# danini/progressive-x

Measured on AMD Instinct MI355X. Metric: residual_evals_per_sec, higher is better.
Workload: dtype f64; 1 GPU; C4 multi-6D-pose points (1e6 2D-3D correspondences, 16 objects, 20% outliers) x metric batch of 2048 pose hypotheses (16 GT + perturbed; weak mode: per GPU), PnP reprojection residual, MSAC + compound-model score, compound instance = 1 model; points=1000000, points_per_gpu=1000000, hypotheses_per_gpu=2048, hypotheses_total=2048, parallelism=1 GPU, exchange=none, device=AMD GPU, 256 CUs (gfx950:sramecc+:xnack-), cu_count=256

## Files before the change

### progressive-x_amd/csrc/capi.hip

```cpp
#include <cmath>
#include <cstdarg>
#include <cstdlib>
#include <cstring>
#include <algorithm>
#include <vector>
#include <cmath>

#include "pgx_internal.h"

namespace pgx {

static thread_local std::string g_err;

int fail(pgx_ctx* ctx, int code, const char* fmt, ...)
{
    char buf[1024];
    va_list ap;
    va_start(ap, fmt);
    vsnprintf(buf, sizeof(buf), fmt, ap);
    va_end(ap);
    if (ctx) ctx->err = buf;
    g_err = buf;
    return code;
}
// ... 130 lines not shown
    if (e != hipSuccess || count <= 0)
        return fail(nullptr, PGX_ERR_HIP, "pgx_create: no HIP device available (%s)",
                    e != hipSuccess ? hipGetErrorString(e) : "device count is 0");
    if (device_id < 0 || device_id >= count)
        return fail(nullptr, PGX_ERR_INVALID, "pgx_create: device %d out of range [0,%d)", device_id, count);
    pgx_ctx* ctx = new pgx_ctx();
    ctx->device = device_id;
    if ((e = hipSetDevice(device_id)) != hipSuccess || (e = hipStreamCreate(&ctx->stream)) != hipSuccess ||
        (e = hipEventCreate(&ctx->ev0)) != hipSuccess || (e = hipEventCreate(&ctx->ev1)) != hipSuccess) {
        int r = fail(nullptr, PGX_ERR_HIP, "pgx_create: HIP init failed: %s", hipGetErrorString(e));
        delete ctx;
        return r;
    }
    hipDeviceProp_t prop;
    if (hipGetDeviceProperties(&prop, device_id) == hipSuccess) ctx->cu_count = prop.multiProcessorCount;
    const char* nf = std::getenv("PGX_NO_FILTER");
    ctx->score_sw.filter_enabled = (nf && nf[0] == '1') ? 0 : ((nf && nf[0] == '2') ? 2 : 1);
    if (const char* ns = std::getenv("PGX_NO_SORT")) ctx->score_sort = (ns[0] == '1') ? 0 : 1;
    if (const char* b = std::getenv("PGX_SP_KD")) { const int v = std::atoi(b); ctx->sp_kd = v < 0 ? 0 : (v > 2 ? 2 : v); }
    if (const char* b = std::getenv("PGX_SETPOINTS_HOST")) ctx->setpoints_host = std::atoi(b) ? 1 : 0;
    if (const char* b = std::getenv("PGX_GC_FLIP")) ctx->route.gc_flip = std::atoi(b) ? 1 : 0;
    if (const char* b = std::getenv("PGX_SCORE_MIRROR")) ctx->score_sw.mirror = std::atoi(b) != 0;
    if (const char* b = std::getenv("PGX_SCORE_NO_CULL")) ctx->score_sw.cull = std::atoi(b) ? 0 : 1;
    if (const char* b = std::getenv("PGX_NO_GROUP")) ctx->group_filter = std::atoi(b) ? 0 : 1;
    if (const char* b = std::getenv("PGX_VERIFY")) ctx->score_sw.verify = std::atoi(b) ? 1 : 0;
    if (const char* b = std::getenv("PGX_MF_TILE")) ctx->route.mf_tile = std::atoi(b) ? 1 : 0;
    if (const char* b = std::getenv("PGX_MF_TILE_BATCH")) ctx->route.mf_tile_batch = std::atoi(b) ? 1 : 0;
    if (const char* b = std::getenv("PGX_MF_REGION")) ctx->route.mf_region = std::atoi(b) ? 1 : 0;
    if (const char* b = std::getenv("PGX_MF_MEMO")) ctx->expansion.mf_memo = std::atoi(b) ? 1 : 0;
    if (const char* b = std::getenv("PGX_MF_DONE_VERIFY")) ctx->expansion.mf_done_verify = std::atoi(b) ? 1 : 0;
    if (const char* b = std::getenv("PGX_MF_XCD")) ctx->mf_xcd = std::atoi(b) ? 1 : 0;
    if (const char* b = std::getenv("PGX_MF_XCD_SEARCH")) ctx->mf_xcd_search = std::atoi(b) ? 1 : 0;
    if (const char* b = std::getenv("PGX_MF_XCD_MIN_DEPTH")) ctx->mf_xcd_min_depth = std::atoi(b);
    if (const char* b = std::getenv("PGX_MF_XCD_MAXN")) ctx->mf_xcd_max_n = std::atoll(b);
    if (const char* b = std::getenv("PGX_MF_SWEEPS")) ctx->mf_sweeps = std::atoi(b);
    if (const char* b = std::getenv("PGX_TILE_MINI")) ctx->tile_mini = std::atoi(b) ? 1 : 0;
    if (const char* b = std::getenv("PGX_TILE_EXPANSION_MAX")) { const int v = std::atoi(b); ctx->route.tile_expansion_max = v < 0 ? 0 : v; }
    if (const char* b = std::getenv("PGX_TILE_MINI_SWEEPS")) { const int v = std::atoi(b); ctx->tile_mini_sweeps = v < 1 ? 1 : v; }
    if (const char* b = std::getenv("PGX_MF_DEBUG")) ctx->tile_debug = std::atoi(b);
    *out = ctx;
    return PGX_OK;
}

void pgx_destroy(pgx_ctx* ctx)
{
    if (!ctx) return;
    (void)hipSetDevice(ctx->device);
    if (ctx->stream) (void)hipStreamSynchronize(ctx->stream);
    comm_free(ctx);
    maxflow_free(ctx);
    tile_free(ctx);
    release(ctx->gorder);
    DevBuf* bufs[] = {&ctx->pts, &ctx->comp, &ctx->pmax, &ctx->pts32, &ctx->perm, &ctx->models, &ctx->pcnt, &ctx->pval, &ctx->psh, &ctx->counts,
                      &ctx->masks, &ctx->g_counts, &ctx->g_values, &ctx->g_shared,
                      &ctx->red_partials, &ctx->red_out, &ctx->dq, &ctx->kmodels, &ctx->labels, &ctx->goff,
                      &ctx->gidx, &ctx->gmult, &ctx->grev, &ctx->scratch, &ctx->fit_scratch, &ctx->pts_s, &ctx->pts32_s,
                      &ctx->pmax_s, &ctx->comp_s, &ctx->pperm, &ctx->gbounds, &ctx->masks_s, &ctx->cull_lists, &ctx->cull_counts, &ctx->gc, &ctx->gc_sel,
                      &ctx->weights, &ctx->stats_buf, &ctx->pts_g, &ctx->p32_g, &ctx->weights_scratch, &ctx->memo_snaps.buf, &ctx->prosac_tops};
    for (DevBuf* b : bufs) release(*b);
    for (DevBuf& b : ctx->slots) release(b);
    release(ctx->h_res);
    release(ctx->h_mirror);
    ctx->h_samples.free();
    ctx->h_models.free();
    if (ctx->h_rb) (void)hipHostFree(ctx->h_rb);
    for (int k = 0; k < 5; ++k) if (ctx->kev[k]) (void)hipEventDestroy(ctx->kev[k]);
    if (ctx->ev0) (void)hipEventDestroy(ctx->ev0);
    if (ctx->ev1) (void)hipEventDestroy(ctx->ev1);
    if (ctx->stream) (void)hipStreamDestroy(ctx->stream);
    delete ctx;
}

const char* pgx_last_error(const pgx_ctx* ctx) { return ctx ? ctx->err.c_str() : g_err.c_str(); }

#define CTX_GUARD(ctx)                                                            \
    do {                                                                          \
        if (!(ctx)) return fail(nullptr, PGX_ERR_INVALID, "ctx is NULL");        \
        hipError_t e_ = hipSetDevice((ctx)->device);                              \
        if (e_ != hipSuccess) return fail(ctx, PGX_ERR_HIP, "hipSetDevice: %s", hipGetErrorString(e_)); \
        (ctx)->rb.clear();                                                        \
// ... 326 lines not shown
}

int pgx_score_algorithmic_bytes(pgx_ctx* ctx, int want_masks, int64_t* bytes, int64_t* pairs)
{
    if (!ctx || ctx->n <= 0 || ctx->batch.resident.M <= 0) return fail(ctx, PGX_ERR_INVALID, "pgx_score_algorithmic_bytes: nothing to score");
    const int64_t M = ctx->batch.resident.M;
    int64_t b = ctx->n * ctx->D * 8 + M * ctx->P * 8 + M * 16;
    if (ctx->batch.last.has_compound) b += ctx->n * 8;
    if (want_masks) b += M * ((ctx->n + 63) / 64) * 8;
    if (bytes) *bytes = b;
    if (pairs) *pairs = ctx->n * M;
    return PGX_OK;
}

int pgx_score_debug_geometry(pgx_ctx* ctx, int what, int value)
{
    CTX_GUARD(ctx);
    switch (what) {
    case 0: if (value < 0 || value > 1024) break; ctx->score_sw.split = value; return PGX_OK;
    case 1: if (value < -1 || value > 1) break; ctx->score_sw.group_xcd = value; return PGX_OK;
    case 2: if (value < 0 || value > 1024 || value % 8) break; ctx->score_sw.nrep = value; return PGX_OK;
    case 3: if (value < 1 || value > 65) break; ctx->score_sw.dense_min = value; return PGX_OK;
    case 4: if (value < 1 || value > 65535) break; ctx->score_sw.cull_segs = value; return PGX_OK;
    }
    return fail(ctx, PGX_ERR_INVALID, "pgx_score_debug_geometry: what = %d, value = %d out of range", what, value);
}

int pgx_score_debug_fetch(pgx_ctx* ctx, int what, void* out, int64_t bytes)
{
    CTX_GUARD(ctx);
    if (!out || bytes <= 0) return fail(ctx, PGX_ERR_INVALID, "pgx_score_debug_fetch: empty destination");
    if (!ctx->point_sort) return fail(ctx, PGX_ERR_INVALID, "pgx_score_debug_fetch: no sorted copies for the resident points");
    const int64_t groups = (ctx->n + 63) / 64, supers = (groups + kSuper - 1) / kSuper;
    if (what == 5) {
        const int64_t want = (int64_t)3 * ctx->batch.resident.Mpad * 8;
        if (bytes != want) return fail(ctx, PGX_ERR_INVALID, "pgx_score_debug_fetch: buffer 5 holds %lld bytes, asked for %lld", (long long)want, (long long)bytes);
        PGX_TRY(ensure(ctx, ctx->g_counts, (size_t)want));
        PGX_TRY(score_acc_export(ctx, (unsigned long long*)ctx->g_counts.p, ctx->stream));
        PGX_TRY(d2h(ctx, out, ctx->g_counts.p, (size_t)bytes));
        PGX_TRY(sync_deliver(ctx));
        return PGX_OK;
    }
    const DevBuf* b = nullptr;
    int64_t have = 0;
    switch (what) {
    case 0: b = &ctx->pperm; have = ctx->n * 4; break;
    case 1: b = &ctx->gbounds; have = (groups + supers) * kGroupRow * 4; break;
    case 2: b = &ctx->pts_g; have = groups * 64 * ctx->D * 8; break;
    case 3: b = &ctx->p32_g; have = groups * 64 * 8 * 4; break;
    case 4: b = &ctx->pts32_s; have = ctx->n * 8 * 4; break;
    default: return fail(ctx, PGX_ERR_INVALID, "pgx_score_debug_fetch: unknown buffer %d", what);
    }
    if (bytes != have) return fail(ctx, PGX_ERR_INVALID, "pgx_score_debug_fetch: buffer %d holds %lld bytes, asked for %lld", what, (long long)have, (long long)bytes);
    PGX_TRY(d2h(ctx, out, b->p, (size_t)bytes));
    PGX_TRY(sync_deliver(ctx));
    return PGX_OK;
}

int pgx_score_profile(pgx_ctx* ctx, int on)
{
    CTX_GUARD(ctx);
    if (on && !ctx->kev[0])
        for (int k = 0; k < 5; ++k) PGX_HIP(ctx, hipEventCreate(&ctx->kev[k]));
    ctx->score_profile = on < 0 ? 0 : (on > 2 ? 2 : on);
    return PGX_OK;
}

int pgx_score_kernel_times(pgx_ctx* ctx, float ms[4])
// ... 443 lines not shown
```

### progressive-x_amd/csrc/pgx_internal.h

```cpp
#pragma once
#include <hip/hip_runtime.h>

#include <cstdint>
#include <cstdio>
#include <string>
#include <vector>

#include "../../include/pgx.h"
#include "expansion_cycle.h"
#include "move_route.h"
#include "residuals.hip.h"
#include "score_plan.h"

namespace pgx {

struct StagedCopy { void* dst; size_t off, bytes; };
struct DevBuf {
    void* p = nullptr;
    size_t cap = 0;
    template <class T> T* as() const { return reinterpret_cast<T*>(p); }
};

struct PinnedBuf { void* p = nullptr; size_t cap = 0; };
struct PinnedStage {
// ... 20 lines not shown
    std::string err;
    int cu_count = 0;

    int model_type = -1, D = 0, P = 0;
    int64_t n = 0;
    pgx::DevBuf pts, comp;
    pgx::DevBuf pmax;
    pgx::DevBuf pts32;
    double umax = 0.0;
    double fscale = 0.0;
    double rmin = 0.0, rmax = __builtin_inf();
    pgx::ScoreSwitches score_sw;
    pgx::DevBuf stats_buf;
    int point_sort = 0;
    int group_filter = 1;
    int comp_dirty = 0;
    pgx::DevBuf pts_s, pts32_s, pmax_s, comp_s, pperm, gbounds, masks_s;
    pgx::DevBuf pts_g, p32_g;
    int setpoints_host = 0;
    double sp_kd_weight = 0.25;
    int sp_kd = 1;
    pgx::DevBuf weights_scratch;
    pgx::DevBuf cull_lists, cull_counts;
    pgx::DevBuf gc;
    pgx::DevBuf gc_sel;

    pgx::ScoreBatch batch;
    int64_t score_global_n = 0;
    pgx::DevBuf models, pcnt, pval, psh, counts, values, shared, masks;
    pgx::DevBuf perm;
    int score_sort = 1;
    pgx::DevBuf g_counts, g_values, g_shared;

    std::vector<pgx::DevBuf> slots;
    pgx::DevBuf red_partials, red_out;

    int L = 0;
    int64_t dq_n = 0;
    pgx::DevBuf dq;
    int64_t dq_max = 0;
    pgx::DevBuf kmodels;
    pgx::DevBuf labels;
    int64_t labels_n = 0;
    pgx::ExpansionState expansion;
    struct MemoSnapshots {
        pgx::DevBuf buf;
// ... 142 lines not shown
```

### progressive-x_amd/csrc/score.hip

```cpp
#include <cmath>
#include <cstdlib>

#include "pgx_internal.h"
#include "score_filters.hip.h"
#include "score_runs.h"

namespace pgx {


template <int MT, bool MASK, int FILT>
__global__ __launch_bounds__(kScoreBlock) void score_kernel(
    const double* __restrict__ pts, int64_t n, const double* __restrict__ models, int M, int Mpad,
    double T2, const double* __restrict__ comp, int has_comp, int64_t chunk,
    const double* __restrict__ pmax, double guard, const float* __restrict__ pts32, double guard32,
    unsigned* __restrict__ pcnt, double* __restrict__ pval, double* __restrict__ psh,
    unsigned long long* __restrict__ masks, int64_t words, const int* __restrict__ perm, int chunks, int xcd_map,
    const float* __restrict__ gbounds)
{
    using R = Residual<MT>;
    int gx = (int)blockIdx.x, gy = (int)blockIdx.y;
    if (xcd_map) {
        const int groups = Mpad / kScoreBlock;
        const int slot = (int)(blockIdx.x >> 3);
        gx = slot % groups;
// ... 140 lines not shown
        }
    }
    static __device__ __forceinline__ LaneT staged(const float (*lds)[64][4], int h)
    {
        LaneT ln;
        float* dst = reinterpret_cast<float*>(&ln);
#pragma unroll
        for (int c = 0; c < kChunks; ++c) {
            if (4 * c + 4 <= kVals) {
                const float4 v = *reinterpret_cast<const float4*>(&lds[c][h][0]);
                dst[4 * c] = v.x; dst[4 * c + 1] = v.y; dst[4 * c + 2] = v.z; dst[4 * c + 3] = v.w;
            } else {
#pragma unroll
                for (int k = 0; k < kVals - 4 * c; ++k) dst[4 * c + k] = lds[c][h][k];
            }
        }
        return ln;
    }
};

constexpr int kCullWaves = 4;
constexpr int kCullTile = 64;

template <int MT>
__global__ __launch_bounds__(64 * kCullWaves) void score_cull_kernel(
    const double* __restrict__ models, int M, double T2, double guard32, const float* __restrict__ gbounds, int groups,
    int gps , int W, unsigned long long* __restrict__ keep, float* __restrict__ hyp32,
    double* __restrict__ models_t ,
    unsigned long long* __restrict__ zero , int64_t zero_words)
{
    using R = Residual<MT>;
    using F32 = Filter32<MT>;
    __shared__ __attribute__((aligned(16))) float s_gb[kCullTile + kCullTile / kSuper][kGroupRow];
    {
        const int64_t nthreads = (int64_t)gridDim.x * gridDim.y * (64 * kCullWaves);
        for (int64_t i = ((int64_t)blockIdx.y * gridDim.x + blockIdx.x) * (64 * kCullWaves) + threadIdx.x; i < zero_words; i += nthreads) zero[i] = 0ull;
    }
    const int lane = (int)(threadIdx.x & 63);
    const int w = (int)blockIdx.x * kCullWaves + (int)(threadIdx.x >> 6), seg = (int)blockIdx.y;
    const int m = w * 64 + lane;
    const bool live = w < W && m < M;
    double mdl[R::P];
#pragma unroll
    for (int k = 0; k < R::P; ++k) mdl[k] = live ? models[(int64_t)m * R::P + k] : __builtin_nan("");
    const typename F32::Lane flane32 = F32::prep(mdl, guard32, T2);
    if (seg == 0 && w < W) {
        HypRow<MT>::store(flane32, hyp32 + (int64_t)m * HypRow<MT>::kStride);
#pragma unroll
        for (int k = 0; k < R::P; ++k) models_t[(int64_t)k * W * 64 + m] = mdl[k];
    }
    const float Tup32 = f32_up(sqrt(T2) * (1.0 + 1.0 / 64.0));
    const int g0 = seg * gps, g1 = g0 + gps < groups ? g0 + gps : groups;
    for (int t0 = g0; t0 < g1; t0 += kCullTile) {
        const int cnt = g1 - t0 < kCullTile ? g1 - t0 : kCullTile;
        __syncthreads();
        const int scnt = (cnt + kSuper - 1) / kSuper;
        for (int e = (int)threadIdx.x; e < cnt * kGroupRow; e += 64 * kCullWaves)
            (&s_gb[0][0])[e] = gbounds[(int64_t)t0 * kGroupRow + e];
        for (int e = (int)threadIdx.x; e < scnt * kGroupRow; e += 64 * kCullWaves)
            (&s_gb[kCullTile][0])[e] = gbounds[((int64_t)groups + t0 / kSuper) * kGroupRow + e];
        __syncthreads();
        if (w >= W) continue;
        for (int sgi = 0; sgi < scnt; ++sgi) {
            const int i0 = sgi * kSuper, i1 = i0 + kSuper < cnt ? i0 + kSuper : cnt;
            float sr[kGroupRow];
#pragma unroll
            for (int k = 0; k < F32::kGroupVals; ++k) sr[k] = s_gb[kCullTile + sgi][k];
            if (__ballot(live && !F32::group_reject(sr, flane32, Tup32)) == 0) {
                if (lane < i1 - i0) keep[(int64_t)(t0 + i0 + lane) * W + w] = 0;
                continue;
            }
            for (int i = i0; i < i1; ++i) {
                float gr[kGroupRow];
#pragma unroll
                for (int k = 0; k < F32::kGroupVals; ++k) gr[k] = s_gb[i][k];
                const unsigned long long bm = __ballot(live && !F32::group_reject(gr, flane32, Tup32));
                if (lane == 0) keep[(int64_t)(t0 + i) * W + w] = bm;
            }
        }
    }
}

__device__ __forceinline__ long long to_fixed(double x)
{
    const double magic = 6755399441055744.0;
    return __double_as_longlong(x + magic) - __double_as_longlong(magic);
}

constexpr int kGroupWaves = 1;

template <int MT, bool MASK, bool STATS = false>
__global__ __launch_bounds__(64 * kGroupWaves) void score_group_kernel(
    const double* __restrict__ pts, const float* __restrict__ pts32, const double* __restrict__ comp, int64_t n, int groups,
    const double* __restrict__ models, int W, double T2, int has_comp, const unsigned long long* __restrict__ keep,
    const float* __restrict__ hyp32, double qscale, unsigned long long* __restrict__ acc ,
    int Mpad, unsigned long long* __restrict__ masks, int64_t words, const int* __restrict__ perm, int split, int xcd_local, const double* __restrict__ models_t,
    unsigned long long* __restrict__ stats ,
    const double* __restrict__ pts_g ,
    const float* __restrict__ p32_g , int nrep, int dense_min)
{
    using R = Residual<MT>;
    using F32 = Filter32<MT>;
    using LaneT = typename F32::Lane;
    using Row = HypRow<MT>;
    const int lane = (int)(threadIdx.x & 63);
    const int wv = 0;
    int g, part;
    if (xcd_local) {
        const int slot = (int)(blockIdx.x >> 3);
        g = (slot / split) * 8 + (int)(blockIdx.x & 7u);
        part = slot % split;
        if (g >= groups) return;
    } else {
        g = (int)blockIdx.x / split;
        part = (int)blockIdx.x % split;
    }
    g = __builtin_amdgcn_readfirstlane(g);
    part = __builtin_amdgcn_readfirstlane(part);
    {
        unsigned long long any = 0;
        for (int w = part; w < W; w += split) any |= keep[(int64_t)g * W + w];
        if (any == 0) return;
    }
    const int64_t j = (int64_t)g * 64 + lane;
    const bool valid = j < n;
    const int64_t jj = valid ? j : n - 1;
    double pt[R::D];
    float p32[8];
    if (pts_g != nullptr) {
#pragma unroll
        for (int q = 0; q < R::D; ++q) pt[q] = pts_g[((int64_t)g * R::D + q) * 64 + lane];
#pragma unroll
        for (int q = 0; q < 8; ++q) p32[q] = 0.0f;
        if constexpr (R::in1 >= R::in0) {
#pragma unroll
            for (int q = 0; q < R::D; ++q) p32[q] = (float)pt[q];
            double pm = 1.0;
#pragma unroll
            for (int q = R::in0; q <= R::in1; ++q) { const double a = fabs(pt[q]); if (!(a <= pm)) pm = a; }
            p32[5] = (float)(pm * 1.000001);
        } else {
#pragma unroll
            for (int q = 0; q < F32::kRowVals; ++q) p32[q] = p32_g[((int64_t)g * 8 + q) * 64 + lane];
        }
    } else {
#pragma unroll
// ... 81 lines not shown
            }
        }
        const unsigned long long bm = __ballot(inl);
        if (bm == 0) return;
        long long val = inl ? to_fixed(sc * qscale) : 0, shq = (inl && has_comp) ? to_fixed(shv * qscale) : 0;
        const bool shares = kTrimDirect ? (has_comp && __ballot(inl && shv != 0.0) != 0) : (has_comp != 0);
        if (shares) {
#pragma unroll
            for (int off = 32; off > 0; off >>= 1) {
                val += __shfl_down(val, off, 64);
                shq += __shfl_down(shq, off, 64);
            }
        } else {
#pragma unroll
            for (int off = 32; off > 0; off >>= 1) val += __shfl_down(val, off, 64);
        }
        if (lane == 0) {
            atomicAdd(&acc[m], (unsigned long long)__popcll(bm));
            atomicAdd(&acc[(int64_t)Mpad + m], (unsigned long long)val);
            if (shares) atomicAdd(&acc[2 * (int64_t)Mpad + m], (unsigned long long)shq);
            if (MASK) masks[(int64_t)perm[m] * words + g] = bm;
        }
    };
    for (int w = part; w < W; w += split) {
        unsigned long long todo = keep[(int64_t)g * W + w];
        if (todo == 0) continue;
        if (STATS) st_steps += (unsigned long long)__popcll(todo);
        __builtin_amdgcn_wave_barrier();
        if ((todo >> lane) & 1ull) {
            const int64_t ml = (int64_t)w * 64 + lane;
            Row::stage(hyp32 + ml * Row::kStride, s_h32[wv], lane);
        }
        __builtin_amdgcn_wave_barrier();
        while (todo != 0) {
            const int h = __builtin_ctzll(todo);
            todo &= todo - 1;
            const int m = w * 64 + h;
            const LaneT ln = Row::staged(s_h32[wv], h);
            const bool cand = valid && !F32::reject(p32, ln, T2d32);
            const unsigned long long cm = __ballot(cand);
            if (cm == 0) continue;
            if (!MASK && __popcll(cm) < dense_min) {
                if (cand) s_queue[wv][qn + __builtin_amdgcn_mbcnt_hi((unsigned)(cm >> 32), __builtin_amdgcn_mbcnt_lo((unsigned)cm, 0u))] =
                    ((unsigned)m << 6) | (unsigned)lane;
                qn += __popcll(cm);
                if (qn >= 64) {
                    __builtin_amdgcn_wave_barrier();
// ... 59 lines not shown
        const bool kept = (todo >> h) & 1ull;
        const LaneT ln = HypRow<MT>::load(hyp32 + (int64_t)m * HypRow<MT>::kStride);
        const bool rej = F32::reject(p32, ln, T2d32);
        c_inl += inl;
        c_cull += inl && !kept;
        c_filt += inl && kept && rej;
    }
#pragma unroll
    for (int off = 32; off > 0; off >>= 1) {
        c_cull += __shfl_down(c_cull, off, 64);
        c_filt += __shfl_down(c_filt, off, 64);
        c_inl += __shfl_down(c_inl, off, 64);
    }
    if (lane == 0) {
        if (c_cull) atomicAdd(&out[0], c_cull);
        if (c_filt) atomicAdd(&out[1], c_filt);
        if (c_inl) atomicAdd(&out[2], c_inl);
    }
}

__global__ __launch_bounds__(256) void score_finish_kernel(const unsigned long long* __restrict__ acc, int M, int Mpad, double qscale,
                                                           const int* __restrict__ perm, long long* __restrict__ counts,
                                                           double* __restrict__ values, double* __restrict__ shared, int nrep,
                                                           long long* __restrict__ mirror )
{
    const int m = (int)(blockIdx.x * 256 + threadIdx.x);
    if (m >= M) return;
    const int o = perm[m];
    unsigned long long c = 0, v = 0, sh = 0;
    for (int r = 0; r < nrep; ++r) {
        const unsigned long long* a = acc + (size_t)r * 3 * (size_t)Mpad;
        c += a[m];
        v += a[(int64_t)Mpad + m];
        sh += a[2 * (int64_t)Mpad + m];
    }
    const double val = (double)(long long)v / qscale, shv = (double)(long long)sh / qscale;
    counts[o] = (long long)c;
    values[o] = val;
    shared[o] = shv;
    if (mirror != nullptr) {
        mirror[m] = (long long)c;
        reinterpret_cast<double*>(mirror)[(int64_t)Mpad + m] = val;
        reinterpret_cast<double*>(mirror)[2 * (int64_t)Mpad + m] = shv;
    }
}

__global__ __launch_bounds__(256) void score_acc_export_kernel(const unsigned long long* __restrict__ acc, int M, int Mpad, int nrep,
                                                               const int* __restrict__ perm, unsigned long long* __restrict__ out)
// ... 110 lines not shown
static int score_group_path(pgx_ctx* ctx, const ScorePlan& pl, double T2, int has_compound, int want_masks, unsigned long long** acc_out)
{
    const int M = ctx->batch.resident.M, Mpad = ctx->batch.resident.Mpad;
    const int groups = pl.groups, W = pl.W, nrep = pl.nrep, split = pl.split, xcd_local = pl.group_xcd ? 1 : 0;
    PGX_TRY(ensure(ctx, ctx->cull_lists, (size_t)groups * W * sizeof(unsigned long long)));
    PGX_TRY(ensure(ctx, ctx->cull_counts, (size_t)Mpad * (HypRow<MT>::kStride * sizeof(float) + (size_t)nrep * 3 * sizeof(long long) + Residual<MT>::P * sizeof(double))));
    float* hyp32 = ctx->cull_counts.as<float>();
    unsigned long long* acc = (unsigned long long*)(ctx->cull_counts.as<char>() + (size_t)Mpad * HypRow<MT>::kStride * sizeof(float));
    double* models_t = (double*)(acc + (size_t)nrep * 3 * (size_t)Mpad);
    const double* pts_g = ctx->pts_g.p ? ctx->pts_g.as<double>() : (const double*)nullptr;
    const float* p32_g = ctx->pts_g.p ? ctx->p32_g.as<float>() : (const float*)nullptr;
    unsigned long long* stats = nullptr;
    if (pl.counters) {
        PGX_TRY(ensure(ctx, ctx->stats_buf, 8 * sizeof(unsigned long long)));
        stats = ctx->stats_buf.as<unsigned long long>();
    }
    long long* mirror = nullptr;
    if (pl.mirror) {
        const size_t need = (size_t)Mpad * 24;
        if (ctx->h_mirror.cap < need) PGX_HIP(ctx, hipStreamSynchronize(ctx->stream));
        PGX_TRY(grow_pinned(ctx, ctx->h_mirror, need, hipHostMallocMapped | hipHostMallocCoherent));
        mirror = (long long*)ctx->h_mirror.p;
    }
    if (ctx->score_profile >= 2) PGX_HIP(ctx, hipEventRecord(ctx->kev[0], ctx->stream));
    hipLaunchKernelGGL((score_cull_kernel<MT>), dim3((unsigned)((W + kCullWaves - 1) / kCullWaves), pl.cull_segs), dim3(64 * kCullWaves), 0,
                       ctx->stream, ctx->models.as<double>(), M, T2, pl.guard32, ctx->gbounds.as<float>(), groups, pl.gps, W,
                       ctx->cull_lists.as<unsigned long long>(), hyp32, models_t, acc, pl.zero_words);
    PGX_HIP(ctx, hipGetLastError());
    if (ctx->score_profile) PGX_HIP(ctx, hipEventRecord(ctx->kev[1], ctx->stream));
    auto group_launch = [&](auto kernel, unsigned long long* masks_s) {
        hipLaunchKernelGGL(kernel, dim3(pl.gblocks), dim3(64 * kGroupWaves), 0, ctx->stream,
                           ctx->pts_s.as<double>(), ctx->pts32_s.as<float>(), ctx->comp_s.as<double>(), ctx->n, groups,
                           ctx->models.as<double>(), W, T2, has_compound, ctx->cull_lists.as<unsigned long long>(), hyp32,
                           pl.qscale, acc, Mpad, masks_s, pl.words, ctx->perm.as<int>(), split, xcd_local, models_t,
                           stats, pts_g, p32_g, nrep, pl.dense_min);
    };
    if (want_masks) {
        PGX_HIP(ctx, hipMemsetAsync(ctx->masks_s.p, 0, (size_t)M * (size_t)pl.words * sizeof(uint64_t), ctx->stream));
        group_launch(score_group_kernel<MT, true>, ctx->masks_s.as<unsigned long long>());
    } else if (pl.counters) {
        PGX_HIP(ctx, hipMemsetAsync(ctx->stats_buf.p, 0, 8 * sizeof(unsigned long long), ctx->stream));
        group_launch(score_group_kernel<MT, false, true>, nullptr);
        if (pl.verify)
            hipLaunchKernelGGL((score_verify_kernel<MT>), dim3((unsigned)groups, (unsigned)W), dim3(64), 0, ctx->stream,
                               ctx->pts_s.as<double>(), ctx->pts32_s.as<float>(), ctx->n, ctx->models.as<double>(), M, W, T2,
                               ctx->cull_lists.as<unsigned long long>(), hyp32, stats + 4);
    } else {
        group_launch(score_group_kernel<MT, false>, nullptr);
    }
    PGX_HIP(ctx, hipGetLastError());
    if (ctx->score_profile) PGX_HIP(ctx, hipEventRecord(ctx->kev[2], ctx->stream));
    if (ctx->score_profile >= 2) PGX_HIP(ctx, hipEventRecord(ctx->kev[4], ctx->stream));
    hipLaunchKernelGGL(score_finish_kernel, dim3((unsigned)((M + 255) / 256)), dim3(256), 0, ctx->stream, acc, M,
                       Mpad, pl.qscale, ctx->perm.as<int>(), ctx->counts.as<long long>(), ctx->values.as<double>(),
                       ctx->shared.as<double>(), nrep, mirror);
    PGX_HIP(ctx, hipGetLastError());
    if (ctx->score_profile >= 2) PGX_HIP(ctx, hipEventRecord(ctx->kev[3], ctx->stream));
    *acc_out = acc;
    return PGX_OK;
}

template <int MT>
static int score_chunked_path(pgx_ctx* ctx, const ScorePlan& pl, double T2, int has_compound, int want_masks)
{
    const int M = ctx->batch.resident.M, Mpad = ctx->batch.resident.Mpad;
    if (ctx->score_profile) PGX_HIP(ctx, hipEventRecord(ctx->kev[0], ctx->stream));
    if constexpr (Filter<MT>::enabled) {
        if (want_masks) {
            if (pl.filter == 2) score_launch_one<MT, true, 2>(ctx, pl, T2, has_compound);
            else if (pl.filter == 1) score_launch_one<MT, true, 1>(ctx, pl, T2, has_compound);
            else score_launch_one<MT, true, 0>(ctx, pl, T2, has_compound);
        } else {
            if (pl.filter == 2) score_launch_one<MT, false, 2>(ctx, pl, T2, has_compound);
            else if (pl.filter == 1) score_launch_one<MT, false, 1>(ctx, pl, T2, has_compound);
            else score_launch_one<MT, false, 0>(ctx, pl, T2, has_compound);
        }
    } else {
        if (want_masks) score_launch_one<MT, true, 0>(ctx, pl, T2, has_compound);
        else score_launch_one<MT, false, 0>(ctx, pl, T2, has_compound);
// ... 212 lines not shown
```

### progressive-x_amd/csrc/score_plan.h

```cpp
#pragma once
#include <cmath>
#include <cstdint>
#include <vector>

namespace pgx {

enum GroupBound : int {
    kBoundBox,
    kBoundBoxAll,
    kBoundBall,
    kBoundVanishing
};

constexpr int kScoreBlock = 256;
constexpr int kSuper = 8;
constexpr int kScoreBlocksPerCu = 64;
constexpr int kScoreXcdMap = 1;
constexpr int kScoreMaxChunk = 65472;
constexpr int kScoreMaxChunks = 65535;

struct ScoreTraits {
    bool filter64 = false;
    bool filter32 = false;
    int bound = kBoundBox;
    bool homography = false;
};

struct ScoreSwitches {
    int filter_enabled{1};
    int cull{1};
    int mirror{1};
    int verify{0};
    int split{0};
    int group_xcd{-1};
    int nrep{0};
    int dense_min{32};
    int cull_segs{256};
};

struct ScorePlan {
    int path = 1;
    int filter = 0;
    double guard = 0.0;
    double guard32 = 0.0;
    int64_t chunk = 0;
    int chunks = 0;
    int64_t words = 0;
    int groups = 0;
    int cull_segs = 0, gps = 0;
    int W = 0;
    int group_xcd = 0;
    int nrep = 0;
    int split = 0;
    unsigned gblocks = 0;
    double qscale = 0.0;
    int64_t zero_words = 0;
    int dense_min = 0;
    bool counters = false;
    bool verify = false;
    bool mirror = false;
};

inline ScorePlan plan_score(const ScoreTraits& tr, const ScoreSwitches& sw, int cu_count, int64_t n, int M, int Mpad, bool ordered,
                            bool point_sort, double T2, double umax, double fscale, int64_t score_global_n, bool want_masks,
                            bool want_counters, int blocks_per_cu = kScoreBlocksPerCu)
{
    (void)M;
    ScorePlan p;
    const double T = std::sqrt(T2);
    bool filt = tr.filter64 && sw.filter_enabled && T > 0.0 && std::isfinite(T) && std::isfinite(umax) && umax <= T * 268435456.0;
    if (filt) {
        p.guard = 4.5 * 1.1102230246251565e-16 * (1.0 + umax + T) * 16777216.0 / T;
        filt = std::isfinite(p.guard);
    }
    bool filt32 = filt && sw.filter_enabled == 1 && umax <= T * 16384.0;
    if (filt32) {
        p.guard32 = 5.5 * 5.9604644775390625e-8 * (1.0 + umax + T) * 1024.0 / T;
        filt32 = std::isfinite(p.guard32) && p.guard32 < 1e30;
    }
    if (tr.bound == kBoundVanishing)
        filt32 = sw.filter_enabled == 1 && T > 0.0 && std::isfinite(T) && T2 < 1e30;
    if (tr.homography)
        filt32 = sw.filter_enabled == 1 && T2 > 1e-24 && T2 < 1e24;
// ... 27 lines not shown

    if (!(tr.filter32 && filt32 && point_sort && sw.cull)) return p;
    p.path = 2;
    p.groups = (int)((n + 63) / 64);
    p.cull_segs = sw.cull_segs;
    p.gps = ((p.groups + p.cull_segs - 1) / p.cull_segs + kSuper - 1) / kSuper * kSuper;
    p.W = Mpad / 64;
    p.group_xcd = sw.group_xcd >= 0 ? sw.group_xcd : (ordered ? 1 : 0);
    p.nrep = sw.nrep > 0 ? sw.nrep : (p.group_xcd ? 8 : 1);
    int lg = 0;
    const int64_t n_scale = score_global_n > n ? score_global_n : n;
    while (((int64_t)1 << lg) < n_scale + 1) ++lg;
    p.qscale = std::ldexp(1.0, 62 - lg < 50 ? 62 - lg : 50);
    p.zero_words = (int64_t)p.nrep * Mpad * 3;
    const bool pose = tr.bound == kBoundBox && !tr.homography;
    const int split_cfg = sw.split > 0 ? sw.split
                          : ((p.group_xcd || pose) ? 5 : ((tr.bound == kBoundVanishing || tr.bound == kBoundBoxAll) ? 16 : 8));
    p.split = split_cfg < p.W ? split_cfg : p.W;
    p.gblocks = p.group_xcd ? (unsigned)((int64_t)((p.groups + 7) / 8) * 8 * p.split) : (unsigned)((int64_t)p.groups * p.split);
    p.dense_min = want_masks ? 65 : sw.dense_min;
    p.counters = want_counters && !want_masks;
    p.verify = p.counters && sw.verify;
    p.mirror = sw.mirror && !want_masks;
    return p;
}

enum class ScoreTable { Ready, None, Changed };
struct ScoreBatch {
    struct Resident {
        int M = 0, Mpad = 0;
        bool ordered = false;
        std::vector<int> perm;
        int64_t generation = 0;
    } resident;
    struct Launch {
        int64_t generation = -1;
        bool has_compound = false, masks = false;
        int64_t words = 0;
        int path = 0, filter = 0;
        unsigned long long* acc = nullptr;
        int nrep = 0;
        double qscale = 0.0;
        bool mirror = false;
    } last;

    void points_changed() { resident.M = 0; resident.Mpad = 0; resident.ordered = false; resident.generation += 1; }
// ... 37 lines not shown
```

### progressive-x_amd/pyprogressivex/_lib.py

```python
import ctypes as C
import os

import numpy as np

os.environ.setdefault("HSA_ENABLE_IPC_MODE_LEGACY", "0")

_HERE = os.path.dirname(os.path.abspath(__file__))
LIB_PATH = os.environ.get("PGX_LIBPGX") or os.path.join(_HERE, "libpgx.so")

LINE2D, HOMOGRAPHY, FUNDAMENTAL, PNP, VANISHING_POINT, HOMOGRAPHY_SYM, PLANE3D = range(7)
SPHERE3D = 8
CIRCLE2D = 10
MODEL_TABLE = {LINE2D: (2, 3, 2, 1), HOMOGRAPHY: (4, 9, 4, 1), FUNDAMENTAL: (4, 9, 7, 3), PNP: (5, 12, 3, 4),
               VANISHING_POINT: (4, 3, 2, 1), HOMOGRAPHY_SYM: (4, 18, 0, 0), PLANE3D: (3, 4, 3, 1), SPHERE3D: (3, 4, 4, 1),
               CIRCLE2D: (2, 3, 3, 1)}
POINT_DIM = {t: row[0] for t, row in MODEL_TABLE.items()}
PARAM_DIM = {t: row[1] for t, row in MODEL_TABLE.items()}
FIXED_ONE = float(1 << 32)
UNIQUE_ID_BYTES = 128

ABI_SYMBOLS = [
    "pgx_version", "pgx_device_count", "pgx_global_error", "pgx_create", "pgx_destroy", "pgx_last_error",
    "pgx_model_dims", "pgx_sync", "pgx_timer_start", "pgx_timer_stop", "pgx_timer_mark", "pgx_timer_elapsed", "pgx_device_info",
    "pgx_set_points", "pgx_set_compound", "pgx_get_compound",
# ... 304 lines not shown
                                                       C.byref(p)), "pgx_score_algorithmic_bytes")
        return b.value, p.value

    def score_inliers(self, row=0):
        if not hasattr(self, "_inl_index") or self._inl_index.shape[0] != self.n:
            self._inl_index = np.empty(self.n, dtype=np.int32)
        cnt = C.c_int64()
        self._ck(self._lib.pgx_score_inliers(self._h, C.c_int(int(row)), _ptr(self._inl_index, C.c_int32), C.byref(cnt)), "pgx_score_inliers")
        return self._inl_index[:cnt.value].astype(np.int64)

    def score_debug_fetch(self, what):
        d = POINT_DIM[self.model_type]
        groups = (self.n + 63) // 64
        supers = (groups + 7) // 8
        spec = {"order": (0, np.int32, (self.n,)), "bounds": (1, np.float32, (groups + supers, 12)),
                "rows64": (2, np.float64, (groups, d, 64)), "rows32": (3, np.float32, (groups, 8, 64)),
                "rows32_sorted": (4, np.float32, (self.n, 8))}[what]
        out = np.empty(spec[2], dtype=spec[1])
        self._ck(self._lib.pgx_score_debug_fetch(self._h, C.c_int(spec[0]), out.ctypes.data_as(C.c_void_p), C.c_int64(out.nbytes)),
                 "pgx_score_debug_fetch")
        return out

    def score_debug_geometry(self, **kw):
        keys = {"split": 0, "group_xcd": 1, "nrep": 2, "dense_min": 3, "cull_segs": 4}
        for k, v in kw.items():
            self._ck(self._lib.pgx_score_debug_geometry(self._h, C.c_int(keys[k]), C.c_int(int(v))), "pgx_score_debug_geometry")

    def score_profile(self, on=1):
        level = 2 if on is True else int(on)
        self._ck(self._lib.pgx_score_profile(self._h, C.c_int(level)), "pgx_score_profile")

    def score_kernel_times(self):
        ms = (C.c_float * 4)()
        self._ck(self._lib.pgx_score_kernel_times(self._h, ms), "pgx_score_kernel_times")
        return float(ms[0]), float(ms[1]), float(ms[2]), float(ms[3])

    def score_stats(self, T2, has_compound=False):
        st = np.zeros(8, dtype=np.int64)
        self._ck(self._lib.pgx_score_stats(self._h, C.c_double(T2), C.c_int(1 if has_compound else 0), _ptr(st, C.c_int64)),
                 "pgx_score_stats")
        return dict(pairs=int(st[0]), group_pairs=int(st[1]), surviving_group_steps=int(st[2]), exact_evaluations=int(st[3]),
                    inlier_pairs=int(st[4]), contradictions=int(st[5]), path={1: "every pair", 2: "cull + group-major"}.get(int(st[6]), "?"),
                    filter={0: "none", 1: "f64", 2: "f32"}.get(int(st[7]), "?"))

    def preference(self, model, T2, slot, want_pref=False):
        m = _f64(model).reshape(-1)
        out = np.empty(self.n, dtype=np.float64) if want_pref else None
        d, a, b = C.c_double(), C.c_double(), C.c_double()
        self._ck(self._lib.pgx_preference(self._h, _ptr(m, C.c_double), C.c_double(T2), C.c_int(int(slot)),
# ... 368 lines not shown
```

Measured before the change: 11650 billion residual-evals/s.

## Schedule group-scoring blocks from cull-built per-XCD work lists ordered by weight

The cull kernel now counts the surviving group-hypothesis steps for each point group and buckets groups into four weight classes in per-XCD work lists using atomics. The group scoring kernel then launches one block per (group, 4-word column) item, taking the heaviest class first, instead of one block per group/split slot that checks for work and returns early. The aim is to stop launching empty blocks and to balance load by scheduling heavy items early. It also adds a waves-per-EU attribute to the cull kernel. The cost is extra atomics and list writes in the cull kernel, a larger grid of mostly small blocks, and counters that the finish kernel must reset. It is enabled by default for pose models.

```diff
diff --git a/progressive-x_amd/csrc/capi.hip b/progressive-x_amd/csrc/capi.hip
--- a/progressive-x_amd/csrc/capi.hip
+++ b/progressive-x_amd/csrc/capi.hip
@@ -176,6 +176,7 @@
     if (const char* b = std::getenv("PGX_GC_FLIP")) ctx->route.gc_flip = std::atoi(b) ? 1 : 0;
     if (const char* b = std::getenv("PGX_SCORE_MIRROR")) ctx->score_sw.mirror = std::atoi(b) != 0;
     if (const char* b = std::getenv("PGX_SCORE_NO_CULL")) ctx->score_sw.cull = std::atoi(b) ? 0 : 1;
+    if (const char* b = std::getenv("PGX_SCORE_WORKLIST")) ctx->score_sw.worklist = std::atoi(b) ? 1 : 0;
     if (const char* b = std::getenv("PGX_NO_GROUP")) ctx->group_filter = std::atoi(b) ? 0 : 1;
     if (const char* b = std::getenv("PGX_VERIFY")) ctx->score_sw.verify = std::atoi(b) ? 1 : 0;
     if (const char* b = std::getenv("PGX_MF_TILE")) ctx->route.mf_tile = std::atoi(b) ? 1 : 0;
@@ -209,7 +210,7 @@
                       &ctx->masks, &ctx->g_counts, &ctx->g_values, &ctx->g_shared,
                       &ctx->red_partials, &ctx->red_out, &ctx->dq, &ctx->kmodels, &ctx->labels, &ctx->goff,
                       &ctx->gidx, &ctx->gmult, &ctx->grev, &ctx->scratch, &ctx->fit_scratch, &ctx->pts_s, &ctx->pts32_s,
-                      &ctx->pmax_s, &ctx->comp_s, &ctx->pperm, &ctx->gbounds, &ctx->masks_s, &ctx->cull_lists, &ctx->cull_counts, &ctx->gc, &ctx->gc_sel,
+                      &ctx->pmax_s, &ctx->comp_s, &ctx->pperm, &ctx->gbounds, &ctx->masks_s, &ctx->cull_lists, &ctx->cull_counts, &ctx->score_wl, &ctx->gc, &ctx->gc_sel,
                       &ctx->weights, &ctx->stats_buf, &ctx->pts_g, &ctx->p32_g, &ctx->weights_scratch, &ctx->memo_snaps.buf, &ctx->prosac_tops};
     for (DevBuf* b : bufs) release(*b);
     for (DevBuf& b : ctx->slots) release(b);
@@ -582,6 +583,10 @@
     case 2: if (value < 0 || value > 1024 || value % 8) break; ctx->score_sw.nrep = value; return PGX_OK;
     case 3: if (value < 1 || value > 65) break; ctx->score_sw.dense_min = value; return PGX_OK;
     case 4: if (value < 1 || value > 65535) break; ctx->score_sw.cull_segs = value; return PGX_OK;
+    case 5: if (value < -1 || value > 1) break; ctx->score_sw.worklist = value; return PGX_OK;
+    case 6: if (value < 1 || value > (1 << 30)) break; ctx->score_sw.wl_t1 = value; return PGX_OK;
+    case 7: if (value < 1 || value > (1 << 30)) break; ctx->score_sw.wl_t2 = value; return PGX_OK;
+    case 8: if (value < 1 || value > (1 << 30)) break; ctx->score_sw.wl_t3 = value; return PGX_OK;
     }
     return fail(ctx, PGX_ERR_INVALID, "pgx_score_debug_geometry: what = %d, value = %d out of range", what, value);
 }
@@ -601,9 +606,23 @@
         PGX_TRY(sync_deliver(ctx));
         return PGX_OK;
     }
+    if (what == 6) {
+        const int64_t want = (int64_t)kWlXcds * kWlClasses * 4;
+        if (bytes != want) return fail(ctx, PGX_ERR_INVALID, "pgx_score_debug_fetch: buffer 6 holds %lld bytes, asked for %lld", (long long)want, (long long)bytes);
+        if (!ctx->batch.current() || ctx->batch.last.path != 2 || !ctx->score_wl_last || !ctx->score_wl.p)
+            return fail(ctx, PGX_ERR_INVALID, "pgx_score_debug_fetch: the last launch did not take its items from work lists");
+        std::vector<unsigned> h((size_t)kWlCountWords);
+        PGX_HIP(ctx, hipMemcpyAsync(h.data(), ctx->score_wl.p, h.size() * sizeof(unsigned), hipMemcpyDeviceToHost, ctx->stream));
+        PGX_HIP(ctx, hipStreamSynchronize(ctx->stream));
+        for (int k = 0; k < kWlXcds * kWlClasses; ++k) ((unsigned*)out)[k] = h[(size_t)k * kWlCountStride + 1];
+        return PGX_OK;
+    }
+    if (what == 7 && !(ctx->batch.current() && ctx->batch.last.path == 2))
+        return fail(ctx, PGX_ERR_INVALID, "pgx_score_debug_fetch: the last launch did not run the cull kernel on the resident batch");
     const DevBuf* b = nullptr;
     int64_t have = 0;
     switch (what) {
+    case 7: b = &ctx->cull_lists; have = groups * (ctx->batch.resident.Mpad / 64) * 8; break;
     case 0: b = &ctx->pperm; have = ctx->n * 4; break;
     case 1: b = &ctx->gbounds; have = (groups + supers) * kGroupRow * 4; break;
     case 2: b = &ctx->pts_g; have = groups * 64 * ctx->D * 8; break;
diff --git a/progressive-x_amd/csrc/pgx_internal.h b/progressive-x_amd/csrc/pgx_internal.h
--- a/progressive-x_amd/csrc/pgx_internal.h
+++ b/progressive-x_amd/csrc/pgx_internal.h
@@ -66,6 +66,9 @@
     int sp_kd = 1;
     pgx::DevBuf weights_scratch;
     pgx::DevBuf cull_lists, cull_counts;
+    pgx::DevBuf score_wl;
+    int score_wl_last = 0;
+    int score_wl_dirty = 0;
     pgx::DevBuf gc;
     pgx::DevBuf gc_sel;
 
diff --git a/progressive-x_amd/csrc/score.hip b/progressive-x_amd/csrc/score.hip
--- a/progressive-x_amd/csrc/score.hip
+++ b/progressive-x_amd/csrc/score.hip
@@ -186,16 +186,20 @@
 constexpr int kCullWaves = 4;
 constexpr int kCullTile = 64;
 
-template <int MT>
-__global__ __launch_bounds__(64 * kCullWaves) void score_cull_kernel(
+template <int MT> constexpr int kCullWavesPerSimd = (MT == kPnP || MT == kHomographySym) ? 7 : 8;
+template <int MT, bool LISTS>
+__global__ __launch_bounds__(64 * kCullWaves) __attribute__((amdgpu_waves_per_eu(kCullWavesPerSimd<MT>))) void score_cull_kernel(
     const double* __restrict__ models, int M, double T2, double guard32, const float* __restrict__ gbounds, int groups,
     int gps , int W, unsigned long long* __restrict__ keep, float* __restrict__ hyp32,
     double* __restrict__ models_t ,
-    unsigned long long* __restrict__ zero , int64_t zero_words)
+    unsigned long long* __restrict__ zero , int64_t zero_words,
+    unsigned* __restrict__ wl , int wl_xb, unsigned wl_cap,
+    unsigned wl_t1, unsigned wl_t2, unsigned wl_t3)
 {
     using R = Residual<MT>;
     using F32 = Filter32<MT>;
     __shared__ __attribute__((aligned(16))) float s_gb[kCullTile + kCullTile / kSuper][kGroupRow];
+    __shared__ unsigned s_wt[kCullWaves][kCullTile];
     {
         const int64_t nthreads = (int64_t)gridDim.x * gridDim.y * (64 * kCullWaves);
         for (int64_t i = ((int64_t)blockIdx.y * gridDim.x + blockIdx.x) * (64 * kCullWaves) + threadIdx.x; i < zero_words; i += nthreads) zero[i] = 0ull;
@@ -224,23 +228,51 @@
         for (int e = (int)threadIdx.x; e < scnt * kGroupRow; e += 64 * kCullWaves)
             (&s_gb[kCullTile][0])[e] = gbounds[((int64_t)groups + t0 / kSuper) * kGroupRow + e];
         __syncthreads();
-        if (w >= W) continue;
-        for (int sgi = 0; sgi < scnt; ++sgi) {
-            const int i0 = sgi * kSuper, i1 = i0 + kSuper < cnt ? i0 + kSuper : cnt;
-            float sr[kGroupRow];
-#pragma unroll
-            for (int k = 0; k < F32::kGroupVals; ++k) sr[k] = s_gb[kCullTile + sgi][k];
-            if (__ballot(live && !F32::group_reject(sr, flane32, Tup32)) == 0) {
-                if (lane < i1 - i0) keep[(int64_t)(t0 + i0 + lane) * W + w] = 0;
-                continue;
-            }
-            for (int i = i0; i < i1; ++i) {
-                float gr[kGroupRow];
-#pragma unroll
-                for (int k = 0; k < F32::kGroupVals; ++k) gr[k] = s_gb[i][k];
-                const unsigned long long bm = __ballot(live && !F32::group_reject(gr, flane32, Tup32));
-                if (lane == 0) keep[(int64_t)(t0 + i) * W + w] = bm;
-            }
+        unsigned steps = 0;
+        if (w < W)
+            for (int sgi = 0; sgi < scnt; ++sgi) {
+                const int i0 = sgi * kSuper, i1 = i0 + kSuper < cnt ? i0 + kSuper : cnt;
+                float sr[kGroupRow];
+#pragma unroll
+                for (int k = 0; k < F32::kGroupVals; ++k) sr[k] = s_gb[kCullTile + sgi][k];
+                if (__ballot(live && !F32::group_reject(sr, flane32, Tup32)) == 0) {
+                    if (lane < i1 - i0) keep[(int64_t)(t0 + i0 + lane) * W + w] = 0;
+                    continue;
+                }
+                for (int i = i0; i < i1; ++i) {
+                    float gr[kGroupRow];
+#pragma unroll
+                    for (int k = 0; k < F32::kGroupVals; ++k) gr[k] = s_gb[i][k];
+                    const unsigned long long bm = __ballot(live && !F32::group_reject(gr, flane32, Tup32));
+                    if (lane == 0) keep[(int64_t)(t0 + i) * W + w] = bm;
+                    if (LISTS) steps = lane == i ? (unsigned)__popcll(bm) : steps;
+                }
+            }
+        if (!LISTS) continue;
+        s_wt[threadIdx.x >> 6][lane] = steps;
+        __syncthreads();
+        if (threadIdx.x >= 64) continue;
+        const int nlive = W - (int)blockIdx.x * kCullWaves < kCullWaves ? W - (int)blockIdx.x * kCullWaves : kCullWaves;
+        unsigned wt = 0;
+        if (lane < cnt)
+            for (int v = 0; v < nlive; ++v) wt += s_wt[v][lane];
+        const int cls = wt != 0 ? wl_class(wt, wl_t1, wl_t2, wl_t3) : -1;
+        unsigned long long mine = 0;
+#pragma unroll
+        for (int c = 0; c < kWlClasses; ++c) {
+            const unsigned long long bc = __ballot(cls == c);
+            if (cls == c) mine = bc & (0x0101010101010101ull << (lane & 7));
+        }
+        const int first = cls >= 0 ? __builtin_ctzll(mine) : lane;
+        const unsigned g = (unsigned)(t0 + lane);
+        const int list = (int)(g & 7u) * kWlClasses + (cls >= 0 ? cls : 0);
+        unsigned base = 0;
+        if (cls >= 0 && lane == first) base = atomicAdd(&wl[list * kWlCountStride], (unsigned)__popcll(mine));
+        base = (unsigned)__shfl((int)base, first, 64);
+        if (cls >= 0) {
+            const unsigned pos = base + __builtin_amdgcn_mbcnt_hi((unsigned)(mine >> 32), __builtin_amdgcn_mbcnt_lo((unsigned)mine, 0u));
+            if (pos < wl_cap)
+                wl[kWlCountWords + (size_t)list * wl_cap + pos] = wl_item(g, blockIdx.x, wl_xb);
         }
     }
 }
@@ -261,7 +293,9 @@
     int Mpad, unsigned long long* __restrict__ masks, int64_t words, const int* __restrict__ perm, int split, int xcd_local, const double* __restrict__ models_t,
     unsigned long long* __restrict__ stats ,
     const double* __restrict__ pts_g ,
-    const float* __restrict__ p32_g , int nrep, int dense_min)
+    const float* __restrict__ p32_g , int nrep, int dense_min,
+    const unsigned* __restrict__ wl ,
+    int wl_xb, unsigned wl_cap)
 {
     using R = Residual<MT>;
     using F32 = Filter32<MT>;
@@ -269,23 +303,39 @@
     using Row = HypRow<MT>;
     const int lane = (int)(threadIdx.x & 63);
     const int wv = 0;
-    int g, part;
-    if (xcd_local) {
-        const int slot = (int)(blockIdx.x >> 3);
-        g = (slot / split) * 8 + (int)(blockIdx.x & 7u);
-        part = slot % split;
-        if (g >= groups) return;
+    int g, w0, w1 = W, wstep = 1;
+    if (wl != nullptr) {
+        const int xcd = (int)(blockIdx.x & 7u);
+        unsigned lc[kWlClasses];
+#pragma unroll
+        for (int c = 0; c < kWlClasses; ++c) lc[c] = wl[wl_count_index(xcd, c)];
+        int cls;
+        unsigned pos;
+        if (!wl_locate(lc[0], lc[1], lc[2], lc[3], blockIdx.x >> 3, &cls, &pos)) return;
+        if (pos >= wl_cap) return;
+        const unsigned item = wl[kWlCountWords + (size_t)(xcd * kWlClasses + cls) * wl_cap + pos];
+        if (wl_item_group(item, wl_xb) >= (unsigned)groups || wl_item_column(item, wl_xb) * kWlItemWords >= (unsigned)W) return;
+        g = (int)wl_item_group(item, wl_xb);
+        w0 = (int)wl_item_column(item, wl_xb) * kWlItemWords;
+        w1 = w0 + kWlItemWords < W ? w0 + kWlItemWords : W;
     } else {
-        g = (int)blockIdx.x / split;
-        part = (int)blockIdx.x % split;
+        if (xcd_local) {
+            const int slot = (int)(blockIdx.x >> 3);
+            g = (slot / split) * 8 + (int)(blockIdx.x & 7u);
+            w0 = slot % split;
+            if (g >= groups) return;
+        } else {
+            g = (int)blockIdx.x / split;
+            w0 = (int)blockIdx.x % split;
+        }
+        wstep = split;
+        unsigned long long any = 0;
+        for (int w = w0; w < W; w += split) any |= keep[(int64_t)g * W + w];
+        if (any == 0) return;
     }
     g = __builtin_amdgcn_readfirstlane(g);
-    part = __builtin_amdgcn_readfirstlane(part);
-    {
-        unsigned long long any = 0;
-        for (int w = part; w < W; w += split) any |= keep[(int64_t)g * W + w];
-        if (any == 0) return;
-    }
+    w0 = __builtin_amdgcn_readfirstlane(w0);
+    w1 = __builtin_amdgcn_readfirstlane(w1);
     const int64_t j = (int64_t)g * 64 + lane;
     const bool valid = j < n;
     const int64_t jj = valid ? j : n - 1;
@@ -413,7 +463,7 @@
             if (MASK) masks[(int64_t)perm[m] * words + g] = bm;
         }
     };
-    for (int w = part; w < W; w += split) {
+    for (int w = w0; w < w1; w += wstep) {
         unsigned long long todo = keep[(int64_t)g * W + w];
         if (todo == 0) continue;
         if (STATS) st_steps += (unsigned long long)__popcll(todo);
@@ -519,8 +569,13 @@
 __global__ __launch_bounds__(256) void score_finish_kernel(const unsigned long long* __restrict__ acc, int M, int Mpad, double qscale,
                                                            const int* __restrict__ perm, long long* __restrict__ counts,
                                                            double* __restrict__ values, double* __restrict__ shared, int nrep,
-                                                           long long* __restrict__ mirror )
-{
+                                                           long long* __restrict__ mirror ,
+                                                           unsigned* __restrict__ wl )
+{
+    if (wl != nullptr && blockIdx.x == 0 && threadIdx.x < kWlXcds * kWlClasses) {
+        wl[threadIdx.x * kWlCountStride + 1] = wl[threadIdx.x * kWlCountStride];
+        wl[threadIdx.x * kWlCountStride] = 0u;
+    }
     const int m = (int)(blockIdx.x * 256 + threadIdx.x);
     if (m >= M) return;
     const int o = perm[m];
@@ -677,18 +732,31 @@
         PGX_TRY(grow_pinned(ctx, ctx->h_mirror, need, hipHostMallocMapped | hipHostMallocCoherent));
         mirror = (long long*)ctx->h_mirror.p;
     }
+    unsigned* wl = nullptr;
+    if (pl.worklist) {
+        const void* before = ctx->score_wl.p;
+        PGX_TRY(ensure(ctx, ctx->score_wl, ((size_t)kWlCountWords + (size_t)kWlXcds * kWlClasses * pl.wl_cap) * sizeof(unsigned)));
+        if (ctx->score_wl.p != before || ctx->score_wl_dirty) PGX_HIP(ctx, hipMemsetAsync(ctx->score_wl.p, 0, kWlCountWords * sizeof(unsigned), ctx->stream));
+        ctx->score_wl_dirty = 1;
+        wl = ctx->score_wl.as<unsigned>();
+    }
     if (ctx->score_profile >= 2) PGX_HIP(ctx, hipEventRecord(ctx->kev[0], ctx->stream));
-    hipLaunchKernelGGL((score_cull_kernel<MT>), dim3((unsigned)((W + kCullWaves - 1) / kCullWaves), pl.cull_segs), dim3(64 * kCullWaves), 0,
-                       ctx->stream, ctx->models.as<double>(), M, T2, pl.guard32, ctx->gbounds.as<float>(), groups, pl.gps, W,
-                       ctx->cull_lists.as<unsigned long long>(), hyp32, models_t, acc, pl.zero_words);
+    auto cull_launch = [&](auto kernel) {
+        hipLaunchKernelGGL(kernel, dim3((unsigned)((W + kCullWaves - 1) / kCullWaves), pl.cull_segs), dim3(64 * kCullWaves), 0,
+                           ctx->stream, ctx->models.as<double>(), M, T2, pl.guard32, ctx->gbounds.as<float>(), groups, pl.gps, W,
+                           ctx->cull_lists.as<unsigned long long>(), hyp32, models_t, acc, pl.zero_words, wl, pl.wl_xbits, pl.wl_cap, pl.wl_t[0],
+                           pl.wl_t[1], pl.wl_t[2]);
+    };
+    if (pl.worklist) cull_launch(score_cull_kernel<MT, true>);
+    else cull_launch(score_cull_kernel<MT, false>);
     PGX_HIP(ctx, hipGetLastError());
     if (ctx->score_profile) PGX_HIP(ctx, hipEventRecord(ctx->kev[1], ctx->stream));
     auto group_launch = [&](auto kernel, unsigned long long* masks_s) {
-        hipLaunchKernelGGL(kernel, dim3(pl.gblocks), dim3(64 * kGroupWaves), 0, ctx->stream,
+        hipLaunchKernelGGL(kernel, dim3(pl.worklist ? pl.wl_grid : pl.gblocks), dim3(64 * kGroupWaves), 0, ctx->stream,
                            ctx->pts_s.as<double>(), ctx->pts32_s.as<float>(), ctx->comp_s.as<double>(), ctx->n, groups,
                            ctx->models.as<double>(), W, T2, has_compound, ctx->cull_lists.as<unsigned long long>(), hyp32,
                            pl.qscale, acc, Mpad, masks_s, pl.words, ctx->perm.as<int>(), split, xcd_local, models_t,
-                           stats, pts_g, p32_g, nrep, pl.dense_min);
+                           stats, pts_g, p32_g, nrep, pl.dense_min, (const unsigned*)wl, pl.wl_xbits, pl.wl_cap);
     };
     if (want_masks) {
         PGX_HIP(ctx, hipMemsetAsync(ctx->masks_s.p, 0, (size_t)M * (size_t)pl.words * sizeof(uint64_t), ctx->stream));
@@ -708,8 +776,10 @@
     if (ctx->score_profile >= 2) PGX_HIP(ctx, hipEventRecord(ctx->kev[4], ctx->stream));
     hipLaunchKernelGGL(score_finish_kernel, dim3((unsigned)((M + 255) / 256)), dim3(256), 0, ctx->stream, acc, M,
                        Mpad, pl.qscale, ctx->perm.as<int>(), ctx->counts.as<long long>(), ctx->values.as<double>(),
-                       ctx->shared.as<double>(), nrep, mirror);
+                       ctx->shared.as<double>(), nrep, mirror, wl);
     PGX_HIP(ctx, hipGetLastError());
+    ctx->score_wl_dirty = 0;
+    ctx->score_wl_last = pl.worklist ? 1 : 0;
     if (ctx->score_profile >= 2) PGX_HIP(ctx, hipEventRecord(ctx->kev[3], ctx->stream));
     *acc_out = acc;
     return PGX_OK;
diff --git a/progressive-x_amd/csrc/score_plan.h b/progressive-x_amd/csrc/score_plan.h
--- a/progressive-x_amd/csrc/score_plan.h
+++ b/progressive-x_amd/csrc/score_plan.h
@@ -2,6 +2,8 @@
 #include <cmath>
 #include <cstdint>
 #include <vector>
+
+#include "score_worklist.h"
 
 namespace pgx {
 
@@ -18,6 +20,8 @@
 constexpr int kScoreXcdMap = 1;
 constexpr int kScoreMaxChunk = 65472;
 constexpr int kScoreMaxChunks = 65535;
+constexpr int kScoreCullSegs = 256;
+constexpr int64_t kWlMaxItems = (int64_t)1 << 22;
 
 struct ScoreTraits {
     bool filter64 = false;
@@ -35,7 +39,9 @@
     int group_xcd{-1};
     int nrep{0};
     int dense_min{32};
-    int cull_segs{256};
+    int cull_segs{kScoreCullSegs};
+    int worklist{-1};
+    int wl_t1{24}, wl_t2{64}, wl_t3{160};
 };
 
 struct ScorePlan {
@@ -59,6 +65,12 @@
     bool counters = false;
     bool verify = false;
     bool mirror = false;
+    bool worklist = false;
+    int wl_columns = 0;
+    int wl_xbits = 0;
+    unsigned wl_cap = 0;
+    unsigned wl_t[3] = {0, 0, 0};
+    unsigned wl_grid = 0;
 };
 
 inline ScorePlan plan_score(const ScoreTraits& tr, const ScoreSwitches& sw, int cu_count, int64_t n, int M, int Mpad, bool ordered,
@@ -132,6 +144,17 @@
     p.counters = want_counters && !want_masks;
     p.verify = p.counters && sw.verify;
     p.mirror = sw.mirror && !want_masks;
+    const int columns = (p.W + kWlItemWords - 1) / kWlItemWords;
+    const int64_t cap = (int64_t)((p.groups + kWlXcds - 1) / kWlXcds) * columns;
+    if (p.group_xcd && sw.split == 0 && sw.cull_segs == kScoreCullSegs && !want_masks && (sw.worklist == 1 || (sw.worklist < 0 && pose)) &&
+        wl_fits(p.groups, columns) && (int64_t)p.groups * columns <= kWlMaxItems) {
+        p.worklist = true;
+        p.wl_columns = columns;
+        p.wl_xbits = wl_xbits(columns);
+        p.wl_cap = (unsigned)cap;
+        p.wl_t[0] = (unsigned)sw.wl_t1; p.wl_t[1] = (unsigned)sw.wl_t2; p.wl_t[2] = (unsigned)sw.wl_t3;
+        p.wl_grid = (unsigned)kWlXcds * p.wl_cap;
+    }
     return p;
 }
 
diff --git a/progressive-x_amd/csrc/score_worklist.h b/progressive-x_amd/csrc/score_worklist.h
--- /dev/null
+++ b/progressive-x_amd/csrc/score_worklist.h
@@ -0,0 +1,48 @@
+#pragma once
+#include <cstdint>
+
+#if defined(__HIPCC__)
+#define PGX_WL_FN __host__ __device__ inline
+#else
+#define PGX_WL_FN inline
+#endif
+
+namespace pgx {
+
+constexpr int kWlXcds = 8;
+constexpr int kWlClasses = 4;
+constexpr int kWlItemWords = 4;
+constexpr int kWlCountStride = 32;
+constexpr int kWlCountWords = kWlXcds * kWlClasses * kWlCountStride;
+
+PGX_WL_FN int wl_count_index(int xcd, int cls) { return (xcd * kWlClasses + cls) * kWlCountStride; }
+
+PGX_WL_FN int wl_class(unsigned weight, unsigned t1, unsigned t2, unsigned t3)
+{
+    return (weight >= t1 ? 1 : 0) + (weight >= t2 ? 1 : 0) + (weight >= t3 ? 1 : 0);
+}
+
+PGX_WL_FN int wl_xbits(int columns)
+{
+    int b = 0;
+    while (((int64_t)1 << b) < columns) ++b;
+    return b;
+}
+PGX_WL_FN bool wl_fits(int64_t groups, int columns) { return columns >= 1 && groups >= 1 && groups <= ((int64_t)1 << (32 - wl_xbits(columns))); }
+PGX_WL_FN uint32_t wl_item(uint32_t g, uint32_t x, int xbits) { return (g << xbits) | x; }
+PGX_WL_FN uint32_t wl_item_group(uint32_t item, int xbits) { return item >> xbits; }
+PGX_WL_FN uint32_t wl_item_column(uint32_t item, int xbits) { return item & (((uint32_t)1 << xbits) - 1u); }
+
+PGX_WL_FN bool wl_locate(uint32_t c0, uint32_t c1, uint32_t c2, uint32_t c3, uint32_t slot, int* cls, uint32_t* pos)
+{
+    if (slot < c3) { *cls = 3; *pos = slot; return true; }
+    slot -= c3;
+    if (slot < c2) { *cls = 2; *pos = slot; return true; }
+    slot -= c2;
+    if (slot < c1) { *cls = 1; *pos = slot; return true; }
+    slot -= c1;
+    if (slot < c0) { *cls = 0; *pos = slot; return true; }
+    return false;
+}
+
+}
diff --git a/progressive-x_amd/pyprogressivex/_lib.py b/progressive-x_amd/pyprogressivex/_lib.py
--- a/progressive-x_amd/pyprogressivex/_lib.py
+++ b/progressive-x_amd/pyprogressivex/_lib.py
@@ -350,9 +350,21 @@
         return out
 
     def score_debug_geometry(self, **kw):
-        keys = {"split": 0, "group_xcd": 1, "nrep": 2, "dense_min": 3, "cull_segs": 4}
+        keys = {"split": 0, "group_xcd": 1, "nrep": 2, "dense_min": 3, "cull_segs": 4, "worklist": 5, "wl_t1": 6, "wl_t2": 7, "wl_t3": 8}
         for k, v in kw.items():
             self._ck(self._lib.pgx_score_debug_geometry(self._h, C.c_int(keys[k]), C.c_int(int(v))), "pgx_score_debug_geometry")
+
+    def score_keep_words(self, Mpad):
+        out = np.empty(((self.n + 63) // 64, Mpad // 64), dtype=np.uint64)
+        self._ck(self._lib.pgx_score_debug_fetch(self._h, C.c_int(7), out.ctypes.data_as(C.c_void_p), C.c_int64(out.nbytes)),
+                 "pgx_score_debug_fetch")
+        return out
+
+    def score_worklist_counts(self):
+        out = np.empty((8, 4), dtype=np.uint32)
+        self._ck(self._lib.pgx_score_debug_fetch(self._h, C.c_int(6), out.ctypes.data_as(C.c_void_p), C.c_int64(out.nbytes)),
+                 "pgx_score_debug_fetch")
+        return out
 
     def score_profile(self, on=1):
         level = 2 if on is True else int(on)
```

After: 12510 billion residual-evals/s, median of 6. 1.07x the previous value.
